# haoheliu/AudioLDM2

Measured on AMD Instinct MI355X. Metric: audio_seconds_per_second, higher is better.
Workload: dtype f32 storage/accumulate; each product = 6 bf16 MFMA partial products of exact 3-part operand splits (fp32-grade); 1 GPU; audioldm2-full: batch 8 prompts/GPU x 1 GPU, 10.24 s @16 kHz, 200 DDIM steps, CFG 3.5, eta 1.0, n_candidates 1; one step = sample_log + VAE decode + HiFi-GAN + D2H of the waveform; synthetic conditioning, random-init weights, host-CPU RNG noise; global_batch=8, parallelism=prompt-sharded replicas x1, weight_broadcast_bytes=0

## Files before the change

audioldm2_amd/csrc/api.hip:

```cpp
#include "common.h"
#include <string.h>

namespace aldm {
static thread_local char g_err[512] = "";
void set_error(const char* fmt, ...) {
    va_list ap;
    va_start(ap, fmt);
    vsnprintf(g_err, sizeof(g_err), fmt, ap);
    va_end(ap);
}
}

extern "C" int aldm_version(void) { return 26; }
extern "C" const char* aldm_last_error(void) { return aldm::g_err; }
```

audioldm2_amd/csrc/igemm.hip:

```cpp
#include "igemm_kernel.h"
#include <algorithm>
#include <atomic>
#include <stdlib.h>

namespace aldm {

int igemm_launch_pre0(int BM, int BN, int kgroups, bool uni, bool w8, dim3 grid, hipStream_t st, const IgemmK& p);
int igemm_launch_pre1(int BM, int BN, int kgroups, bool uni, bool w8, dim3 grid, hipStream_t st, const IgemmK& p);
int igemm_launch_pre2(int BM, int BN, int kgroups, bool uni, bool w8, dim3 grid, hipStream_t st, const IgemmK& p);
int igemm_launch_pre3(int BM, int BN, int kgroups, bool uni, bool w8, dim3 grid, hipStream_t st, const IgemmK& p);
int igemm_launch_pre4(int BM, int BN, int kgroups, bool uni, bool w8, dim3 grid, hipStream_t st, const IgemmK& p);
int igemm_launch_bx_pre0(int BM, int BN, int kgroups, bool uni, bool w8, dim3 grid, hipStream_t st, const IgemmK& p);
int igemm_launch_bx_pre1(int BM, int BN, int kgroups, bool uni, bool w8, dim3 grid, hipStream_t st, const IgemmK& p);
int igemm_launch_bx_pre2(int BM, int BN, int kgroups, bool uni, bool w8, dim3 grid, hipStream_t st, const IgemmK& p);
int igemm_launch_bx_pre3(int BM, int BN, int kgroups, bool uni, bool w8, dim3 grid, hipStream_t st, const IgemmK& p);

int igemm_launch_dma(int BM, int BN, int nst, int parts, bool f16, dim3 grid, hipStream_t st, const IgemmK& p);
bool igemm_dma_config_ok(int BM, int BN, int nst, int parts);
#ifdef ALDM_TEST_HOOKS
extern std::atomic<int> g_debug_drop_product;
#endif
int igemm_launch_dma_ws(int BM, int BN, int nst, int parts, int blocks, hipStream_t st, const IgemmK& p);
bool igemm_dma_ws_config_ok(int BM, int BN, int nst, int parts);
int igemm_dma_ws_blocks_per_cu(int BM, int BN, int nst, int parts);
// ... 58 lines not shown
        split_store4_out(d, d.out_split, orow, d.out_split_c, n, r);
    }
}

__global__ void pack_weight_kernel(const float* __restrict__ src, float* __restrict__ dst, int N,
                                   int Cin, int KH, int KW, int Kg, int Npad) {
    const int64_t total = (int64_t)Kg * Npad * 4;
    for (int64_t i = blockIdx.x * (int64_t)blockDim.x + threadIdx.x; i < total;
         i += (int64_t)gridDim.x * blockDim.x) {
        const int j = i & 3;
        const int n = (i >> 2) % Npad;
        const int kg = (i >> 2) / Npad;
        const int k = kg * 4 + j;
        float v = 0.f;
        if (n < N && k < KH * KW * Cin) {
            const int tap = k / Cin, ci = k - tap * Cin;
            const int kh = tap / KW, kw = tap - kh * KW;
            v = src[(((int64_t)n * Cin + ci) * KH + kh) * KW + kw];
        }
        dst[i] = v;
    }
}

__global__ void pack_weight_tr_kernel(const float* __restrict__ src, float* __restrict__ dst, int N,
                                      int Cin, int KWfull, int T, int phase, int stride, int Kg,
                                      int Npad) {
    const int64_t total = (int64_t)Kg * Npad * 4;
    for (int64_t i = blockIdx.x * (int64_t)blockDim.x + threadIdx.x; i < total;
         i += (int64_t)gridDim.x * blockDim.x) {
        const int jj = i & 3;
        const int n = (i >> 2) % Npad;
        const int kg = (i >> 2) / Npad;
        const int k = kg * 4 + jj;
        float v = 0.f;
        if (n < N && k < T * Cin) {
            const int kwp = k / Cin, ci = k - kwp * Cin;
            const int j = T - 1 - kwp;
            const int kk = phase + j * stride;
            if (kk < KWfull) v = src[((int64_t)ci * N + n) * KWfull + kk];
        }
        dst[i] = v;
    }
}

__global__ void pack_kn_kernel(const float* __restrict__ src, float* __restrict__ dst, int K, int N,
                               int lds, int Kg, int Npad, int64_t stride_src, int64_t stride_dst) {
// ... 98 lines not shown
    return mask < 0 ? default_wave8_mask() : mask;
}

static thread_local int g_force_mma = 0;
extern "C" int aldm_igemm_mma(int mode) {
    const int prev = g_force_mma;
    if (mode >= 0 && mode <= 2) g_force_mma = mode;
    return prev;
}

static std::atomic<int> g_epi_forms{-1};
static int epi_forms_on() {
    static const int env_on = [] {
        const char* e = getenv("ALDM_EPI_FORMS");
        return (e && e[0] == '0' && e[1] == 0) ? 0 : 1;
    }();
    const int v = g_epi_forms.load(std::memory_order_relaxed);
    return v < 0 ? env_on : v;
}
extern "C" int aldm_igemm_epilogue_forms(int on) {
    const int prev = epi_forms_on();
    g_epi_forms.store(on == 0 || on == 1 ? on : -1, std::memory_order_relaxed);
    return prev;
}

static int plan_epilogue_form(const IgemmK& p, int BM, int BN) {
    const aldm_igemm_desc& d = p.d;
    if (!epi_forms_on() || !p.dma || d.a_fmt != ALDM_FMT_BF16) return ALDM_EPI_FORM_GENERIC;
    const bool inst = p.ws == 0   ? igemm_dma_form_ok(BM, BN, p.nst, d.split_parts)
                      : p.ws == 2 ? igemm_dma_lw_form_ok(BM, BN, p.nst, d.split_parts)
                      : p.ws == 4 ? igemm_dma_halo_form_ok(BM, BN, p.nst, p.ws_blocks, d.split_parts, p.os_rows)
                                  : false;
    if (!inst) return ALDM_EPI_FORM_GENERIC;
    if (d.epi_mode != ALDM_EPI_PLAIN || p.splits != 1 || d.act != ALDM_ACT_NONE || d.alpha != 1.0f || d.accumulate ||
        d.out_mul > 0 || d.batch != 1)
        return ALDM_EPI_FORM_GENERIC;
    auto al16 = [](const void* q) { return (reinterpret_cast<uintptr_t>(q) & 15) == 0; };
    if ((d.N & 3) != 0 || (d.ldo & 3) != 0 || (d.stride_o & 3) != 0 || !al16(d.out) || !al16(d.res) || !al16(d.bias) ||
        !al16(d.rowbias) || (d.rowbias && (p.rb_ld & 3) != 0))
        return ALDM_EPI_FORM_GENERIC;
    if (d.out_split && (d.out_split_fmt != ALDM_FMT_BF16 || d.out_split_parts != d.split_parts)) return ALDM_EPI_FORM_GENERIC;
#ifdef ALDM_TEST_HOOKS
    if (g_debug_drop_product.load(std::memory_order_relaxed)) return ALDM_EPI_FORM_GENERIC;
#endif
    if (d.res && d.rowbias) return ALDM_EPI_FORM_GENERIC;
    return d.res ? ALDM_EPI_FORM_RES : (d.rowbias ? ALDM_EPI_FORM_ROWBIAS : ALDM_EPI_FORM_PLAIN);
// ... 40 lines not shown
    if (d.rowbias || d.accumulate || d.act != ALDM_ACT_NONE) return false;
    auto al16 = [](const void* q) { return (reinterpret_cast<uintptr_t>(q) & 15) == 0; };
    if ((d.N & 3) != 0 || (d.ldo & 3) != 0 || !al16(d.out) || !al16(d.res)) return false;
    return true;
}

static int dma_halo_chunks(const IgemmK& p, int BM) {
    const aldm_igemm_desc& d = p.d;
    if (d.KH != 3 || d.KW != 3 || d.SH != 1 || d.SW != 1 || d.PH != 1 || d.PW != 1 || d.DH != 1 || d.DW != 1) return 0;
    if (d.up_h != 1 || d.up_w != 1 || d.OH != d.H || d.OW != d.W || d.out_mul > 0 || d.batch > 1) return 0;
    if (d.W <= 0 || (d.W & (d.W - 1)) != 0 || BM % d.W != 0 || p.OHW % BM != 0) return 0;
    return ((BM / d.W + 2) * d.W + 15) / 16;
}

static bool tile_supported(int BM, int BN) {
    return (BM == 128 && (BN == 128 || BN == 64 || BN == 32)) || (BM == 64 && (BN == 128 || BN == 64));
}

static int igemm_prepare(const aldm_igemm_desc* dd, IgemmK& p, int& BM, int& BN) {
    ALDM_CHECK(dd != nullptr, "aldm_igemm: null descriptor");
    p.d = *dd;
    aldm_igemm_desc& d = p.d;
    p.epi_form = ALDM_EPI_FORM_GENERIC;
    ALDM_CHECK((d.x1 || d.a_split) && d.w && (d.out || d.out_split), "aldm_igemm: null x1/w/out");
    if (!d.x1) d.x1 = reinterpret_cast<const float*>(d.a_split);
    if (d.split_parts == 0) d.split_parts = 3;
    ALDM_CHECK(d.split_parts == 2 || d.split_parts == 3, "aldm_igemm: split_parts must be 0 / 3 or 2");
    if (d.out_split_parts == 0) d.out_split_parts = d.split_parts;
    ALDM_CHECK(d.out_split_parts == 2 || d.out_split_parts == 3, "aldm_igemm: out_split_parts must be 0, 2 or 3");
    ALDM_CHECK(d.a_fmt == ALDM_FMT_BF16 || (d.a_fmt == ALDM_FMT_F16 && d.a_split != nullptr && d.split_parts == 2 && d.acc_scale > 0.0f),
               "aldm_igemm: a_fmt = ALDM_FMT_F16 needs a pre-split operand (a_split), 2-part images and acc_scale > 0");
    if (d.a_fmt == ALDM_FMT_BF16) d.acc_scale = 1.0f;
    ALDM_CHECK(d.out_split_fmt == ALDM_FMT_BF16 ||
                   (d.out_split_fmt == ALDM_FMT_F16 && d.out_split_scale > 0.0f &&
                    (d.epi_mode == ALDM_EPI_QKV ? (d.k_split != nullptr && d.vt_split != nullptr && d.vt_scale > 0.0f) : d.out_split != nullptr)),
               "aldm_igemm: out_split_fmt = ALDM_FMT_F16 needs out_split (QKV: k_split, vt_split and vt_scale) and out_split_scale > 0");
    if (d.out_split_fmt == ALDM_FMT_F16) d.out_split_parts = 2;
    if (!d.x2) d.C2 = 0;
    if (d.pix1 == 0) d.pix1 = d.C1;
    if (d.pix2 == 0) d.pix2 = d.C2;
    if (d.up_h == 0) d.up_h = 1;
    if (d.up_w == 0) d.up_w = 1;
    if (d.batch == 0) d.batch = 1;
    p.Cin = d.C1 + d.C2;
    ALDM_CHECK(d.C1 > 0 && d.C1 % 4 == 0 && d.C2 % 4 == 0,
               "aldm_igemm: C1=%d/C2=%d must be multiples of 4", d.C1, d.C2);
// ... 364 lines not shown
    if (bn) *bn = BN;
    if (flops) *flops = 2ll * p.M * p.d.N * p.d.K * p.d.batch;
    if (splits) *splits = p.splits;
    if (kgroups) *kgroups = p.kgroups;
    if (mma) *mma = p.bx ? ALDM_MMA_BF16X6 : ALDM_MMA_F32;
    return 0;
}

extern "C" int aldm_igemm_plan_stages(const aldm_igemm_desc* dd) {
    IgemmK p;
    int BM, BN;
    if (igemm_prepare(dd, p, BM, BN)) return -1;
    if (p.dma && p.ws == 4) return 400 + (BM == 128 && p.ws_blocks == 4 ? 10 : 0) + p.nst;
    return p.dma ? p.nst + 100 * p.ws : 0;
}

extern "C" int aldm_igemm_plan_epilogue(const aldm_igemm_desc* dd) {
    IgemmK p;
    int BM, BN;
    if (igemm_prepare(dd, p, BM, BN)) return -1;
    return plan_epilogue_form(p, BM, BN);
}

extern "C" int64_t aldm_igemm_ws_floats(const aldm_igemm_desc* dd) {
    if (!dd) return 0;
    aldm_igemm_desc t = *dd;
    t.ws = reinterpret_cast<float*>(uintptr_t(16));
    t.ws_floats = INT64_MAX;
    IgemmK p;
    int BM, BN;
    if (igemm_prepare(&t, p, BM, BN)) return 0;
    return p.splits > 1 ? (int64_t)p.d.batch * p.splits * p.M * p.d.N : 0;
}

extern "C" int aldm_igemm(const aldm_igemm_desc* dd, void* stream) {
    IgemmK p;
    int BM, BN;
    int rc = igemm_prepare(dd, p, BM, BN);
    if (rc) return rc;
    p.epi_form = plan_epilogue_form(p, BM, BN);
    const aldm_igemm_desc& d = p.d;
    dim3 grid((unsigned)(p.tiles_m * p.tiles_n), (unsigned)p.splits, (unsigned)d.batch);
    hipStream_t st = (hipStream_t)stream;
    const int pre = p.pre;
    const bool uni = p.OHW % BM == 0;
    const int env_w8 = g_wave8_mask < 0 ? default_wave8_mask() : g_wave8_mask;
// ... 96 lines not shown
    hipStream_t st = (hipStream_t)stream;
    if (!transposed) {
        const int K = KH * KW * Cin;
        const int Kg = (K + 3) / 4;
        const int64_t total = (int64_t)Kg * Npad * 4;
        const int blocks = (int)std::min<int64_t>(cdiv64(total, 256), 4096);
        hipLaunchKernelGGL(pack_weight_kernel, dim3(blocks), dim3(256), 0, st, src, dst, N, Cin, KH,
                           KW, Kg, Npad);
    } else {
        ALDM_CHECK(KH == 1 && stride > 0 && phase >= 0 && phase < stride,
                   "aldm_pack_weight: bad transposed args");
        const int T = (KW + stride - 1) / stride;
        const int K = T * Cin;
        const int Kg = (K + 3) / 4;
        const int64_t total = (int64_t)Kg * Npad * 4;
        const int blocks = (int)std::min<int64_t>(cdiv64(total, 256), 4096);
        hipLaunchKernelGGL(pack_weight_tr_kernel, dim3(blocks), dim3(256), 0, st, src, dst, N, Cin,
                           KW, T, phase, stride, Kg, Npad);
    }
    ALDM_LAUNCH_CHECK("aldm_pack_weight");
    return 0;
}

extern "C" int aldm_pack_kn(const float* src, float* dst, int K, int N, int lds, int batch,
                            int64_t stride_src, int64_t stride_dst, void* stream) {
    ALDM_CHECK(src && dst && K > 0 && N > 0 && lds >= N && batch > 0, "aldm_pack_kn: bad args");
    const int Npad = (N + 31) / 32 * 32;
    const int Kg = (K + 3) / 4;
    const int64_t total = (int64_t)Kg * Npad * 4;
    const int blocks = (int)std::min<int64_t>(cdiv64(total, 256), 4096);
    hipLaunchKernelGGL(pack_kn_kernel, dim3(blocks, batch), dim3(256), 0, (hipStream_t)stream, src,
                       dst, K, N, lds, Kg, Npad, stride_src, stride_dst);
    ALDM_LAUNCH_CHECK("aldm_pack_kn");
    return 0;
}
```

audioldm2_amd/lib.py:

```python
from __future__ import annotations

import ctypes as C
import os

_HERE = os.path.dirname(os.path.abspath(__file__))
LIB_PATH = os.environ.get("ALDM_LIB_PATH") or os.path.join(_HERE, "libaldm_hip.so")
ABI_VERSION = 26

ACT_NONE, ACT_SILU, ACT_LRELU, ACT_TANH, ACT_LOGCLAMP, ACT_GELU, ACT_GELU_TANH = range(7)
B_PACKED, B_NT = 0, 1
EPI_PLAIN, EPI_GEGLU, EPI_QKV = 0, 1, 2
GN_CHUNKED, GN_FUSED, GN_FUSED_SPLIT = 0, 1, 2
FMT_BF16, FMT_F16 = 0, 1
EPI_FORM_GENERIC, EPI_FORM_PLAIN, EPI_FORM_ROWBIAS, EPI_FORM_RES = range(4)


class IgemmDesc(C.Structure):

    _fields_ = [
        ("x1", C.c_void_p), ("x2", C.c_void_p),
        ("C1", C.c_int32), ("C2", C.c_int32),
        ("pix1", C.c_int32), ("pix2", C.c_int32),
        ("B", C.c_int32), ("H", C.c_int32), ("W", C.c_int32),
        ("up_h", C.c_int32), ("up_w", C.c_int32),
        ("KH", C.c_int32), ("KW", C.c_int32), ("SH", C.c_int32), ("SW", C.c_int32),
        ("PH", C.c_int32), ("PW", C.c_int32), ("DH", C.c_int32), ("DW", C.c_int32),
        ("OH", C.c_int32), ("OW", C.c_int32),
        ("pre_scale", C.c_void_p), ("pre_shift", C.c_void_p),
        ("pre_act", C.c_int32), ("pre_slope", C.c_float),
        ("w", C.c_void_p),
        ("b_mode", C.c_int32), ("ldb", C.c_int32),
        ("K", C.c_int32), ("N", C.c_int32),
        ("bias", C.c_void_p), ("rowbias", C.c_void_p), ("res", C.c_void_p), ("out", C.c_void_p),
        ("ldo", C.c_int32), ("act", C.c_int32), ("act_slope", C.c_float), ("alpha", C.c_float),
        ("accumulate", C.c_int32),
        ("out_mul", C.c_int32), ("out_off", C.c_int32), ("out_len", C.c_int32),
        ("batch", C.c_int32),
        ("stride_x", C.c_int64), ("stride_w", C.c_int64), ("stride_o", C.c_int64),
        ("rowbias_ld", C.c_int32), ("epi_mode", C.c_int32),
        ("ws", C.c_void_p), ("ws_floats", C.c_int64),
        ("hint_bm", C.c_int32), ("hint_bn", C.c_int32), ("hint_splits", C.c_int32), ("hint_kgroups", C.c_int32),
        ("w_split", C.c_void_p), ("hint_mma", C.c_int32), ("hint_stages", C.c_int32),
        ("a_split", C.c_void_p), ("out_split", C.c_void_p), ("out_split_c", C.c_int32), ("split_parts", C.c_int32),
        ("out_split_act", C.c_int32), ("out_split_slope", C.c_float),
        ("k_split", C.c_void_p), ("vt_split", C.c_void_p), ("qkv_c", C.c_int32), ("qkv_rows", C.c_int32),
        ("a_fmt", C.c_int32), ("acc_scale", C.c_float), ("out_split_parts", C.c_int32),
        ("out_split_fmt", C.c_int32), ("out_split_scale", C.c_float), ("vt_scale", C.c_float),
    ]


MAX_WINDOWS = 32


class WindowStarts(C.Structure):

    _fields_ = [("n", C.c_int), ("s", C.c_int * MAX_WINDOWS)]


MAX_ROWS = 64


class WindowRows(C.Structure):

    _fields_ = [("n", C.c_int), ("s", C.c_int * MAX_ROWS)]


_SIGS = {
    "aldm_version": (C.c_int, []),
    "aldm_last_error": (C.c_char_p, []),
    "aldm_igemm": (C.c_int, [C.POINTER(IgemmDesc), C.c_void_p]),
    "aldm_igemm_plan": (C.c_int, [C.POINTER(IgemmDesc), C.POINTER(C.c_int), C.POINTER(C.c_int),
                                  C.POINTER(C.c_int64), C.POINTER(C.c_int), C.POINTER(C.c_int),
                                  C.POINTER(C.c_int)]),
    "aldm_igemm_ws_floats": (C.c_int64, [C.POINTER(IgemmDesc)]),
    "aldm_igemm_plan_stages": (C.c_int, [C.POINTER(IgemmDesc)]),
    "aldm_igemm_plan_epilogue": (C.c_int, [C.POINTER(IgemmDesc)]),
    "aldm_igemm_epilogue_forms": (C.c_int, [C.c_int]),
    "aldm_igemm_force": (None, [C.c_int, C.c_int, C.c_int, C.c_int]),
    "aldm_igemm_force_stages": (None, [C.c_int]),
    "aldm_igemm_wave8_mask": (C.c_int, [C.c_int]),
    "aldm_split_image_bytes": (C.c_int64, [C.c_int64, C.c_int, C.c_int]),
    "aldm_split_rows": (C.c_int, [C.c_void_p, C.c_void_p, C.c_int, C.c_int, C.c_int64, C.c_int, C.c_void_p, C.c_void_p,
                                  C.c_int, C.c_void_p, C.c_void_p, C.c_int, C.c_void_p]),
    "aldm_split_rows_act": (C.c_int, [C.c_void_p, C.c_void_p, C.c_int, C.c_int, C.c_int64, C.c_int, C.c_void_p, C.c_void_p,
                                      C.c_int, C.c_float, C.c_void_p, C.c_void_p, C.c_int, C.c_void_p]),
    "aldm_layernorm_split": (C.c_int, [C.c_void_p, C.c_void_p, C.c_void_p, C.c_int, C.c_int, C.c_void_p, C.c_void_p,
                                       C.c_float, C.c_int, C.c_void_p]),
    "aldm_attention_d32_split": (C.c_int, [C.c_void_p, C.c_void_p, C.c_void_p, C.c_void_p, C.c_void_p, C.c_int, C.c_int,
                                           C.c_int, C.c_int, C.c_int, C.c_int, C.c_int, C.c_int, C.c_int,
                                           C.c_void_p, C.c_float, C.c_void_p]),
    "aldm_split_bytes_parts": (C.c_int64, [C.c_int, C.c_int, C.c_int]),
    "aldm_pack_split_bf16_parts": (C.c_int, [C.c_void_p, C.c_void_p, C.c_int, C.c_int, C.c_int, C.c_void_p]),
    "aldm_pack_split_f16": (C.c_int, [C.c_void_p, C.c_void_p, C.c_int, C.c_int, C.c_float, C.c_void_p]),
    "aldm_split_rows_f16": (C.c_int, [C.c_void_p, C.c_void_p, C.c_int, C.c_int, C.c_int64, C.c_int, C.c_void_p, C.c_void_p,
                                      C.c_int, C.c_float, C.c_void_p, C.c_void_p, C.c_int, C.c_float, C.c_void_p]),
    "aldm_groupnorm_split_f16": (C.c_int, [C.c_void_p, C.c_void_p, C.c_int, C.c_int, C.c_int, C.c_int, C.c_int, C.c_float,
                                           C.c_void_p, C.c_void_p, C.c_int, C.c_void_p, C.c_void_p, C.c_void_p, C.c_void_p,
                                           C.c_void_p, C.c_int, C.c_float, C.c_void_p]),
    "aldm_layernorm_split_f16": (C.c_int, [C.c_void_p, C.c_void_p, C.c_void_p, C.c_int, C.c_int, C.c_void_p, C.c_void_p,
                                           C.c_float, C.c_float, C.c_void_p]),
# ... 199 lines not shown
```

audioldm2_amd/ops.py:

```python
from __future__ import annotations

import ctypes as C
import json
import os
from dataclasses import dataclass
from typing import List, Optional, Sequence, Tuple

import torch

from . import lib as _l
from .lib import (ACT_GELU, ACT_GELU_TANH, ACT_LOGCLAMP, ACT_LRELU, ACT_NONE, ACT_SILU, ACT_TANH, B_NT, B_PACKED,
                  IgemmDesc)


def _stream() -> int:
    return torch.cuda.current_stream().cuda_stream


def _p(t: Optional[torch.Tensor]):
    return None if t is None else t.data_ptr()


def _chk(t: torch.Tensor, name: str):
    if not (t.is_cuda and t.dtype == torch.float32 and t.is_contiguous()):
# ... 88 lines not shown


def _norm_f16_scale(gamma: torch.Tensor, beta: Optional[torch.Tensor], n: int) -> float:
    import math
    return _pow2_scale(math.sqrt(float(n)) * _absmax_cached(gamma) + _absmax_cached(beta))


@dataclass
class Packed:
    data: torch.Tensor
    N: int
    Cin: int
    KH: int
    KW: int
    bias: Optional[torch.Tensor] = None
    split: Optional[torch.Tensor] = None
    split2: Optional[torch.Tensor] = None
    split16: Optional[torch.Tensor] = None
    w_scale: float = 0.0
    cmax: Optional[float] = None
    bmax: float = 0.0
    geglu: bool = False
    halves: Optional[tuple] = None

    @property
    def K(self) -> int:
        return self.KH * self.KW * self.Cin

    def out_bound(self, rn: float) -> float:
        if self.cmax is None:
            if torch.cuda.is_current_stream_capturing():
                raise RuntimeError("f16x3: a weight's column norms must be known before graph capture (run one eager step)")
            npad = self.data.numel() // (4 * ((self.K + 3) // 4))
            self.cmax = float(self.data.view(-1, npad, 4).double().pow(2).sum((0, 2)).max().sqrt())
            self.bmax = 0.0 if self.bias is None else float(self.bias.abs().max())
        return rn * self.cmax + self.bmax

    def geglu_bound(self, rn: float, rt: float) -> Tuple[float, float]:
        import math
        assert self.geglu
        if self.halves is None:
            if torch.cuda.is_current_stream_capturing():
                raise RuntimeError("f16x3: a weight's column norms must be known before graph capture (run one eager step)")
            npad = self.data.numel() // (4 * ((self.K + 3) // 4))
            cn = self.data.view(-1, npad, 4).double().pow(2).sum((0, 2)).sqrt()[:self.N].view(-1, 2, 32)
            b = torch.zeros(self.N, device=self.data.device) if self.bias is None else self.bias
            b = b.double().view(-1, 2, 32)
            self.halves = tuple((float(cn[:, j].max()), float(cn[:, j].median()), float(b[:, j].abs().max()),
                                 float(b[:, j].pow(2).mean().sqrt())) for j in range(2))
        bound, typ = 1.0, 1.0
# ... 145 lines not shown


def _workspace(lib, d: IgemmDesc, device) -> None:
    need = lib.aldm_igemm_ws_floats(C.byref(d))
    if need <= 0:
        return
    key = (device.index if device.index is not None else torch.cuda.current_device(), WS_SLOT)
    buf = _ws.get(key)
    if buf is None or buf.numel() < need:
        if torch.cuda.is_current_stream_capturing():
            return
        if buf is not None:
            _ws_retired.append(buf)
        buf = torch.empty(max(need, 8 << 20), device=device, dtype=torch.float32)
        _ws[key] = buf
    d.ws = buf.data_ptr()
    d.ws_floats = buf.numel()


_TUNE_FIELDS = ("B", "H", "W", "C1", "C2", "pix1", "up_h", "up_w", "KH", "KW", "SH", "SW", "PH", "PW", "DH", "DW",
                "OH", "OW", "N", "b_mode", "batch", "epi_mode", "out_mul")
_TUNED = None
TUNE_LOG = None


def tune_key(d: IgemmDesc) -> str:
    return ",".join(str(getattr(d, f)) for f in _TUNE_FIELDS) + f",{_pre_mode(d)}" + \
        (("," + ("dma2" if d.split_parts == 2 else "dma")) if d.a_split else "")


def _tuned_table(bx=False):
    global _TUNED
    if _TUNED is None:
        _TUNED = {False: {}, True: {}, "dma": {}, "dma2": {}}
        if os.environ.get("ALDM_NO_TUNING", "0") != "1":
            for mode, name in ((False, "mi355x_igemm.json"), (True, "mi355x_igemm_bf16x6.json"),
                               ("dma", "mi355x_igemm_dma.json"), ("dma2", "mi355x_igemm_dma_bf16x3.json")):
                path = os.path.join(os.environ.get("ALDM_TUNING_DIR", ""), name)
                if not (os.environ.get("ALDM_TUNING_DIR") and os.path.exists(path)):
                    path = os.path.join(os.path.dirname(os.path.abspath(__file__)), "tuning", name)
                if os.path.exists(path):
                    with open(path) as f:
                        _TUNED[mode] = {k: v[:5] if mode is True else v[:4] for k, v in json.load(f)["entries"].items()}
    return _TUNED[bx]


def _set_split_operand(d: IgemmDesc, x: "SplitT", pw: "Packed", so: Optional["SplitT"] = None) -> None:
    d.a_split = x.data_ptr()
    d.split_parts = x.parts
    if x.fmt == "f16":
# ... 125 lines not shown
    global _wave8_mask
    _wave8_mask = mask
    return _l.load().aldm_igemm_wave8_mask(mask)


def _npad(n: int) -> int:
    return (n + 31) // 32 * 32


def pack_conv(weight: torch.Tensor, bias: Optional[torch.Tensor] = None) -> Packed:
    w = weight.detach().to(device="cuda", dtype=torch.float32).contiguous()
    if w.dim() == 2:
        N, Cin, KH, KW = w.shape[0], w.shape[1], 1, 1
    elif w.dim() == 3:
        N, Cin, KH, KW = w.shape[0], w.shape[1], 1, w.shape[2]
    else:
        N, Cin, KH, KW = w.shape
    K = KH * KW * Cin
    dst = torch.empty(((K + 3) // 4) * _npad(N) * 4, device="cuda", dtype=torch.float32)
    lib = _l.load()
    _l.check(lib.aldm_pack_weight(w.data_ptr(), dst.data_ptr(), N, Cin, KH, KW, 0, 0, 1, _stream()),
             "pack_weight")
    b = None if bias is None else bias.detach().to(device="cuda", dtype=torch.float32).contiguous()
    return Packed(dst, N, Cin, KH, KW, b)


def pack_geglu(weight: torch.Tensor, bias: Optional[torch.Tensor]) -> Packed:
    two_inner = weight.shape[0]
    inner = two_inner // 2
    assert weight.dim() == 2 and two_inner % 64 == 0
    g = torch.arange(inner // 32).view(-1, 1, 1)
    j = torch.arange(2).view(1, -1, 1)
    l = torch.arange(32).view(1, 1, -1)
    perm = (j * inner + g * 32 + l).reshape(-1).to(weight.device)
    pw = pack_conv(weight.detach()[perm], None if bias is None else bias.detach()[perm])
    pw.geglu = True
    return pw


def linear_geglu(x, pw: Packed, split_out: Optional[str] = None, gate_act: int = ACT_NONE,
                 out: Optional[torch.Tensor] = None):
    is_split = isinstance(x, SplitT)
    if not is_split:
        _chk(x, "linear_geglu.x")
    shp = x.shape
    M = (x.rows if is_split else x.numel() // shp[-1])
    assert shp[-1] == pw.Cin and pw.KH == 1 and pw.KW == 1 and pw.N % 64 == 0
# ... 168 lines not shown
        OH = (VH + 2 * pad[0] - dil[0] * (pw.KH - 1) - 1) // stride[0] + 1
        OW = (VW + 2 * pad[1] - dil[1] * (pw.KW - 1) - 1) // stride[1] + 1
    else:
        OH, OW = out_hw
    N = pw.N
    if remap is not None:
        out_mul, out_off, out_len = remap
        oshape = (B, 1, out_len, N)
    else:
        out_mul = out_off = out_len = 0
        oshape = (B, OH, OW, N)
    if split_out == "only":
        assert out is None and not accumulate
    elif out is None:
        assert not accumulate
        out = torch.empty(oshape, device=x.device, dtype=torch.float32)
    else:
        _chk(out, "conv.out")
        assert out.numel() == oshape[0] * oshape[1] * oshape[2] * oshape[3], (out.shape, oshape)
    so = SplitT.empty(oshape, x.device) if split_out else None
    if bias is None and use_pw_bias:
        bias = pw.bias
    d = IgemmDesc()
    if is_split:
        _set_split_operand(d, x, pw, so)
    else:
        d.x1 = x.data_ptr(); d.split_parts = so.parts if so is not None else 3
    d.x2 = _p(x2)
    d.C1 = C1; d.C2 = C2; d.pix1 = 0; d.pix2 = 0
    d.B = B; d.H = H; d.W = W; d.up_h = up[0]; d.up_w = up[1]
    d.KH = pw.KH; d.KW = pw.KW; d.SH = stride[0]; d.SW = stride[1]
    d.PH = pad[0]; d.PW = pad[1]; d.DH = dil[0]; d.DW = dil[1]
    d.OH = OH; d.OW = OW
    if pre is not None:
        d.pre_scale = pre[0].data_ptr(); d.pre_shift = pre[1].data_ptr()
    d.pre_act = pre_act; d.pre_slope = pre_slope
    d.w = pw.data.data_ptr(); d.b_mode = B_PACKED; d.ldb = 0
    if not is_split:
        d.w_split = pw.split_ptr(3)
    d.K = pw.K; d.N = N
    d.bias = _p(bias); d.rowbias = _p(rowbias); d.res = _p(res); d.out = _p(out)
    if so is not None:
        d.out_split = so.data_ptr(); d.out_split_c = N
        d.out_split_act = split_act; d.out_split_slope = split_slope
    if rowbias is not None:
        if not (rowbias.dim() == 2 and rowbias.stride(1) == 1 and rowbias.shape == (B, N)):
            raise RuntimeError("conv.rowbias: need a [B, N] fp32 view with unit inner stride")
        d.rowbias_ld = rowbias.stride(0)
    d.ldo = N; d.act = act; d.act_slope = act_slope; d.alpha = alpha
    d.accumulate = 1 if accumulate else 0
    d.out_mul = out_mul; d.out_off = out_off; d.out_len = out_len
    d.batch = 1
    _igemm(d, "igemm(conv)")
    if split_out == "only":
        return so
    return (out.view(oshape), so) if split_out else out.view(oshape)


def linear(x, pw: Packed, **kw):
    shp = x.shape
    if isinstance(x, SplitT):
        M = x.rows
        y = conv(x.view(1, 1, M, shp[-1]), pw, **kw)
    else:
        M = x.numel() // shp[-1]
        y = conv(x.reshape(1, 1, M, shp[-1]), pw, **kw)
    oshape = (*shp[:-1], pw.N)
    if isinstance(y, tuple):
        return y[0].view(oshape), y[1].view(oshape)
    return y.view(oshape)


def _view3(t: torch.Tensor, name: str):
    if not (t.is_cuda and t.dtype == torch.float32 and t.dim() == 3 and t.stride(2) == 1):
        raise RuntimeError(f"{name}: need a [Z, R, D] fp32 CUDA view with unit inner stride")
# ... 990 lines not shown
```

audioldm2_amd/unet.py:

```python
from __future__ import annotations

from typing import List, Optional

import torch
import torch.nn as nn

import os

from . import ops
from .ops import ACT_NONE, ACT_SILU

PRESPLIT_ATTENTION = os.environ.get("ALDM_ATTN_PRESPLIT", "1") != "0" and "ALDM_ATTN_MMA" not in os.environ


class ResBlock(nn.Module):

    def __init__(self, channels, emb_channels, dropout, out_channels=None):
        super().__init__()
        self.channels = channels
        self.out_channels = out_channels or channels
        self.in_layers = nn.Sequential(nn.GroupNorm(32, channels), nn.SiLU(),
                                       nn.Conv2d(channels, self.out_channels, 3, padding=1))
        self.emb_layers = nn.Sequential(nn.SiLU(), nn.Linear(emb_channels, self.out_channels))
        self.out_layers = nn.Sequential(nn.GroupNorm(32, self.out_channels), nn.SiLU(), nn.Dropout(p=dropout),
# ... 390 lines not shown
    def collect_context_kv(self, contexts):
        out = []
        for m in self.modules():
            if isinstance(m, BasicTransformerBlock) and m._kv:
                for ctx, _ver, kv, fold in m._kv:
                    if any(ctx is c for c in contexts):
                        out.append((m, ctx, kv, fold))
        return out

    def refresh_context_kv(self, entries):
        n = 0
        for m, ctx, kv, fold in entries:
            pk = m._prepare()
            ops.linear(ctx, pk["kv2"], out=kv)
            if fold is not None:
                fold.prepare(kv, pk["wq2"], pk["wout2"])
            m._kv = [(ctx, ctx._version, kv, fold)] + [c for c in (m._kv or ()) if c[2] is not kv][:1]
            n += 1
        return n

    def _prepare(self):
        if self._pk is None:
            f = lambda t: t.detach().float().cuda().contiguous()
            rbs = [m for m in self.modules() if isinstance(m, ResBlock)]
            off = 0
            for m in rbs:
                m._emb_slice = slice(off, off + m.out_channels)
                off += m.out_channels
            self._pk = dict(
                emb_all=ops.pack_conv(torch.cat([m.emb_layers[1].weight for m in rbs], 0),
                                      torch.cat([m.emb_layers[1].bias for m in rbs], 0)),
                te0=ops.pack_conv(self.time_embed[0].weight, self.time_embed[0].bias),
                te2=ops.pack_conv(self.time_embed[2].weight, self.time_embed[2].bias),
                film=ops.pack_conv(self.film_emb.weight, self.film_emb.bias)
                if self.use_extra_film_by_concat else None,
                gn=(f(self.out[0].weight), f(self.out[0].bias)),
                out=ops.pack_conv(self.out[2].weight, self.out[2].bias),
            )
        return self._pk

    def _shared_prefix_end(self, context_list):
        if self.use_extra_film_by_concat:
            return None
        for bi, blk in enumerate(self.input_blocks):
            st = 0
            for li, layer in enumerate(blk):
                if isinstance(layer, SpatialTransformer):
                    if st >= 1 and st - 1 < len(context_list) and context_list[st - 1] is not None:
                        return bi, li
                    st += 1
        return None

    @torch.no_grad()
    def forward(self, x, timesteps=None, y=None, context_list=None, context_attn_mask_list=None, cfg_shared=False, **kwargs):
        assert (y is not None) == self.use_extra_film_by_concat, \
            "must specify y if and only if the model is class-conditional or film embedding conditional"
        if not x.is_cuda:
            raise RuntimeError("UNetModel(HIP) runs on the MI355X only; there is no CPU path")
        pk = self._prepare()
        context_list = [c.float().contiguous() if c is not None else None for c in (context_list or [])]
        mask_list = list(context_attn_mask_list or [])
        div = self._shared_prefix_end(context_list) if cfg_shared else None
        B = x.shape[0]
        if cfg_shared:
            assert timesteps.shape[0] in (B, 2 * B) and all(c is None or c.shape[0] == 2 * B for c in context_list), \
                "cfg_shared: x [B, ...] once, contexts for the 2B rows [uncond ; cond]"
            timesteps = timesteps[:B]
            if div is None:
                x = x.repeat(2, 1, 1, 1)
                timesteps = timesteps.repeat(2)
        t_emb = ops.timestep_embedding(timesteps, self.model_channels)
        emb = ops.linear(ops.linear(t_emb, pk["te0"], act=ACT_SILU), pk["te2"])
        if self.use_extra_film_by_concat:
            emb = torch.cat([emb, ops.linear(y.float().contiguous(), pk["film"])], dim=-1).contiguous()
        emb_rows = ops.linear(emb, pk["emb_all"], pre_act=ACT_SILU)
        emb = _EmbSlices(emb_rows)
        h = ops.nchw_to_nhwc(x.float().contiguous())
        hs = []
        if div is None:
            for module in self.input_blocks:
                h = module.run(h, emb, context_list, mask_list)
                hs.append(h)
        else:
            dup = lambda t: t.repeat(2, *([1] * (t.dim() - 1)))
            emb_half, emb = emb, _EmbSlices(dup(emb_rows))
            for bi, module in enumerate(self.input_blocks):
                if bi < div[0]:
                    h = module.run(h, emb_half, context_list, mask_list)
                elif bi == div[0]:
                    h = module.run(h, emb_half, context_list, mask_list, hi=div[1])
                    h = module.run(dup(h), emb, context_list, mask_list, lo=div[1])
                else:
                    h = module.run(h, emb, context_list, mask_list)
                hs.append(h)
        h = self.middle_block.run(h, emb, context_list, mask_list)
        for module in self.output_blocks:
            skip = hs.pop()
            if skip.shape[0] != h.shape[0]:
# ... 6 lines not shown
```

include/aldm_hip.h:

```cpp
#ifndef ALDM_HIP_H
#define ALDM_HIP_H

#include <stdint.h>

#ifdef __cplusplus
extern "C" {
#endif

int aldm_version(void);
const char* aldm_last_error(void);

enum {
    ALDM_ACT_NONE = 0,
    ALDM_ACT_SILU = 1,
    ALDM_ACT_LRELU = 2,
    ALDM_ACT_TANH = 3,
    ALDM_ACT_LOGCLAMP = 4,
    ALDM_ACT_GELU = 5,
    ALDM_ACT_GELU_TANH = 6
};

enum { ALDM_EPI_PLAIN = 0, ALDM_EPI_GEGLU = 1, ALDM_EPI_QKV = 2 };

enum {
// ... 37 lines not shown
    float* ws;
    int64_t ws_floats;
    int32_t hint_bm, hint_bn, hint_splits;
    int32_t hint_kgroups;
    const void* w_split;
    int32_t hint_mma;
    int32_t hint_stages;
    const void* a_split;
    void* out_split;
    int32_t out_split_c;
    int32_t split_parts;
    int32_t out_split_act;
    float out_split_slope;
    void* k_split;
    void* vt_split;
    int32_t qkv_c;
    int32_t qkv_rows;
    int32_t a_fmt;
    float acc_scale;
    int32_t out_split_parts;
    int32_t out_split_fmt;
    float out_split_scale;
    float vt_scale;
} aldm_igemm_desc;

int aldm_igemm(const aldm_igemm_desc* d, void* stream);
int64_t aldm_igemm_ws_floats(const aldm_igemm_desc* d);
enum { ALDM_FMT_BF16 = 0, ALDM_FMT_F16 = 1 };
int aldm_igemm_plan(const aldm_igemm_desc* d, int* bm, int* bn, int64_t* flops, int* splits, int* kgroups,
                    int* mma);
int aldm_igemm_plan_stages(const aldm_igemm_desc* d);
enum { ALDM_EPI_FORM_GENERIC = 0, ALDM_EPI_FORM_PLAIN = 1, ALDM_EPI_FORM_ROWBIAS = 2, ALDM_EPI_FORM_RES = 3 };
int aldm_igemm_plan_epilogue(const aldm_igemm_desc* d);
int aldm_igemm_epilogue_forms(int on);
void aldm_igemm_force(int bm, int bn, int splits, int kgroups);
void aldm_igemm_force_stages(int stages);
int aldm_igemm_wave8_mask(int mask);
int aldm_igemm_mma(int mode);
#ifdef ALDM_TEST_HOOKS
int aldm_debug_drop_product(int on);
#endif
int64_t aldm_split_bytes(int K, int N);
int aldm_pack_split_bf16(const float* packed, void* dst, int K, int N, void* stream);
int64_t aldm_split_bytes_parts(int K, int N, int parts);
int aldm_pack_split_bf16_parts(const float* packed, void* dst, int K, int N, int parts, void* stream);
int aldm_pack_split_f16(const float* packed, void* dst, int K, int N, float scale, void* stream);

int64_t aldm_split_image_bytes(int64_t rows, int C, int parts);
int aldm_split_rows(const float* x1, const float* x2, int C1, int C2, int64_t rows, int P, const float* scale,
                    const float* shift, int act, void* dst, void* dst_raw, int parts, void* stream);
int aldm_split_rows_act(const float* x1, const float* x2, int C1, int C2, int64_t rows, int P, const float* scale,
                        const float* shift, int act, float slope, void* dst, void* dst_raw, int parts, void* stream);
int aldm_split_rows_f16(const float* x1, const float* x2, int C1, int C2, int64_t rows, int P, const float* scale,
                        const float* shift, int act, float slope, void* dst, void* dst_raw, int raw_parts, float f16_scale,
                        void* stream);

int aldm_pack_weight(const float* src, float* dst, int N, int Cin, int KH, int KW,
// ... 164 lines not shown
```

Baseline: 19.55 audio-s/s.

## Merge width-2 3x3 convolutions into 1-wide GEMMs with column-merged weights

For 3x3 stride-1 convs whose input width is 2, the two output columns are folded into the output-channel dimension. A new packed weight image of shape 6*Cin by 2N (zero padding taps dropped) lets the implicit GEMM run as a 1-wide conv with half the K-padding waste and doubled N. The per-ResBlock embedding projection is duplicated to produce [B,2N] row biases that match the merged layout. It adds extra weight images and a geometry blacklist, and requires a warm-up eager step before graph capture.

```diff
diff --git a/audioldm2_amd/csrc/api.hip b/audioldm2_amd/csrc/api.hip
--- a/audioldm2_amd/csrc/api.hip
+++ b/audioldm2_amd/csrc/api.hip
@@ -11,5 +11,5 @@
 }
 }
 
-extern "C" int aldm_version(void) { return 26; }
+extern "C" int aldm_version(void) { return 27; }
 extern "C" const char* aldm_last_error(void) { return aldm::g_err; }
diff --git a/audioldm2_amd/csrc/igemm.hip b/audioldm2_amd/csrc/igemm.hip
--- a/audioldm2_amd/csrc/igemm.hip
+++ b/audioldm2_amd/csrc/igemm.hip
@@ -104,6 +104,30 @@
     }
 }
 
+__host__ __device__ inline int64_t wmerge_src_index(int N, int Cin, int dy, int xin, int ci, int xout, int co) {
+    (void)N;
+    const int kw = xin - xout + 1;
+    return (((int64_t)co * Cin + ci) * 3 + dy) * 3 + kw;
+}
+
+__global__ void pack_weight_wmerge_kernel(const float* __restrict__ src, float* __restrict__ dst, int N, int Cin, int Kg, int Npad) {
+    const int64_t total = (int64_t)Kg * Npad * 4;
+    for (int64_t i = blockIdx.x * (int64_t)blockDim.x + threadIdx.x; i < total; i += (int64_t)gridDim.x * blockDim.x) {
+        const int j = i & 3;
+        const int n = (i >> 2) % Npad;
+        const int kg = (i >> 2) / Npad;
+        const int k = kg * 4 + j;
+        float v = 0.f;
+        if (n < 2 * N && k < 6 * Cin) {
+            const int tap = k / Cin, ci = k - tap * Cin;
+            const int dy = tap >> 1, xin = tap & 1;
+            const int xout = n / N, co = n - xout * N;
+            v = src[wmerge_src_index(N, Cin, dy, xin, ci, xout, co)];
+        }
+        dst[i] = v;
+    }
+}
+
 __global__ void pack_weight_tr_kernel(const float* __restrict__ src, float* __restrict__ dst, int N,
                                       int Cin, int KWfull, int T, int phase, int stride, int Kg,
                                       int Npad) {
@@ -248,6 +272,57 @@
     const int prev = epi_forms_on();
     g_epi_forms.store(on == 0 || on == 1 ? on : -1, std::memory_order_relaxed);
     return prev;
+}
+
+static std::atomic<int> g_conv_wmerge{-1};
+static int conv_wmerge_on() {
+    static const int env_on = [] {
+        const char* e = getenv("ALDM_CONV_WMERGE");
+        return (e && e[0] == '0' && e[1] == 0) ? 0 : 1;
+    }();
+    const int v = g_conv_wmerge.load(std::memory_order_relaxed);
+    return v < 0 ? env_on : v;
+}
+extern "C" int aldm_conv_wmerge(int on) {
+    const int prev = conv_wmerge_on();
+    g_conv_wmerge.store(on == 0 || on == 1 ? on : -1, std::memory_order_relaxed);
+    return prev;
+}
+
+static bool wmerge_geometry_wins(int H, int C2x, int N2x) {
+    (void)H;
+    if (N2x == 1280 && (C2x == 768 || C2x == 1280 || C2x == 2048 || C2x == 2560)) return false;
+    return true;
+}
+extern "C" int aldm_conv_wmerge_wins(int H, int C, int N) {
+    return conv_wmerge_on() && H > 0 && C > 0 && N > 0 && C % 32 == 0 && wmerge_geometry_wins(H, 2 * C, 2 * N) ? 1 : 0;
+}
+
+static bool wmerge_applies(const aldm_igemm_desc& d) {
+    if (!conv_wmerge_on() || !d.a_split || !d.wm_split || d.a_fmt != ALDM_FMT_BF16) return false;
+    if (d.W != 2 || d.OW != 2 || d.KH != 3 || d.KW != 3 || d.SH != 1 || d.SW != 1 || d.DH != 1 || d.DW != 1 || d.PW != 1) return false;
+    if (d.up_h > 1 || d.up_w > 1 || d.OH != d.H + 2 * d.PH - 2 || d.OH < 1) return false;
+    if (d.x2 || d.C2 != 0 || d.pre_scale || d.pre_shift || d.pre_act != ALDM_ACT_NONE) return false;
+    if (d.out_mul > 0 || d.accumulate || d.out_split || d.epi_mode != ALDM_EPI_PLAIN || d.batch > 1) return false;
+    if (d.C1 <= 0 || d.C1 % 32 != 0 || (d.pix1 != 0 && d.pix1 != d.C1) || d.K != 9 * d.C1 || d.N <= 0 || d.ldo != d.N) return false;
+    if (d.b_mode != ALDM_B_PACKED || (reinterpret_cast<uintptr_t>(d.wm_split) & 15) != 0) return false;
+    if (d.bias && !d.wm_bias) return false;
+    if (d.rowbias && (!d.wm_rowbias2 || d.rowbias_ld < 2 * d.N)) return false;
+    return wmerge_geometry_wins(d.H, 2 * d.C1, 2 * d.N);
+}
+
+static void wmerge_rewrite(aldm_igemm_desc& d) {
+    d.K = 6 * d.C1;
+    d.C1 *= 2;
+    d.pix1 = 0;
+    d.W = 1;
+    d.OW = 1;
+    d.KW = 1;
+    d.PW = 0;
+    d.N *= 2;
+    d.ldo = d.N;
+    d.bias = d.bias ? d.wm_bias : nullptr;
+    d.w_split = d.wm_split;
 }
 
 static int plan_epilogue_form(const IgemmK& p, int BM, int BN) {
@@ -334,6 +409,7 @@
     p.d = *dd;
     aldm_igemm_desc& d = p.d;
     p.epi_form = ALDM_EPI_FORM_GENERIC;
+    if (wmerge_applies(d)) wmerge_rewrite(d);
     ALDM_CHECK((d.x1 || d.a_split) && d.w && (d.out || d.out_split), "aldm_igemm: null x1/w/out");
     if (!d.x1) d.x1 = reinterpret_cast<const float*>(d.a_split);
     if (d.split_parts == 0) d.split_parts = 3;
@@ -744,6 +820,19 @@
     return plan_epilogue_form(p, BM, BN);
 }
 
+extern "C" int aldm_igemm_plan_wmerge(const aldm_igemm_desc* dd) {
+    IgemmK p;
+    int BM, BN;
+    if (igemm_prepare(dd, p, BM, BN)) return -1;
+    return wmerge_applies(*dd) ? 1 : 0;
+}
+
+extern "C" int64_t aldm_conv_wmerge_index(int N, int Cin, int dy, int xin, int ci, int xout, int co) {
+    if (N <= 0 || Cin <= 0 || dy < 0 || dy > 2 || xin < 0 || xin > 1 || xout < 0 || xout > 1 || ci < 0 || ci >= Cin || co < 0 || co >= N)
+        return -1;
+    return wmerge_src_index(N, Cin, dy, xin, ci, xout, co);
+}
+
 extern "C" int64_t aldm_igemm_ws_floats(const aldm_igemm_desc* dd) {
     if (!dd) return 0;
     aldm_igemm_desc t = *dd;
@@ -886,6 +975,17 @@
     return 0;
 }
 
+extern "C" int aldm_pack_weight_wmerge(const float* src, float* dst, int N, int Cin, void* stream) {
+    ALDM_CHECK(src && dst && N > 0 && Cin > 0 && (int64_t)N * Cin * 9 < (1ll << 31), "aldm_pack_weight_wmerge: bad args");
+    const int Npad = (2 * N + 31) / 32 * 32;
+    const int Kg = (6 * Cin + 3) / 4;
+    const int64_t total = (int64_t)Kg * Npad * 4;
+    const int blocks = (int)std::min<int64_t>(cdiv64(total, 256), 4096);
+    hipLaunchKernelGGL(pack_weight_wmerge_kernel, dim3(blocks), dim3(256), 0, (hipStream_t)stream, src, dst, N, Cin, Kg, Npad);
+    ALDM_LAUNCH_CHECK("aldm_pack_weight_wmerge");
+    return 0;
+}
+
 extern "C" int aldm_pack_kn(const float* src, float* dst, int K, int N, int lds, int batch,
                             int64_t stride_src, int64_t stride_dst, void* stream) {
     ALDM_CHECK(src && dst && K > 0 && N > 0 && lds >= N && batch > 0, "aldm_pack_kn: bad args");
diff --git a/audioldm2_amd/lib.py b/audioldm2_amd/lib.py
--- a/audioldm2_amd/lib.py
+++ b/audioldm2_amd/lib.py
@@ -5,7 +5,7 @@
 
 _HERE = os.path.dirname(os.path.abspath(__file__))
 LIB_PATH = os.environ.get("ALDM_LIB_PATH") or os.path.join(_HERE, "libaldm_hip.so")
-ABI_VERSION = 26
+ABI_VERSION = 27
 
 ACT_NONE, ACT_SILU, ACT_LRELU, ACT_TANH, ACT_LOGCLAMP, ACT_GELU, ACT_GELU_TANH = range(7)
 B_PACKED, B_NT = 0, 1
@@ -46,6 +46,7 @@
         ("k_split", C.c_void_p), ("vt_split", C.c_void_p), ("qkv_c", C.c_int32), ("qkv_rows", C.c_int32),
         ("a_fmt", C.c_int32), ("acc_scale", C.c_float), ("out_split_parts", C.c_int32),
         ("out_split_fmt", C.c_int32), ("out_split_scale", C.c_float), ("vt_scale", C.c_float),
+        ("wm_split", C.c_void_p), ("wm_bias", C.c_void_p), ("wm_rowbias2", C.c_int32),
     ]
 
 
@@ -76,6 +77,11 @@
     "aldm_igemm_plan_stages": (C.c_int, [C.POINTER(IgemmDesc)]),
     "aldm_igemm_plan_epilogue": (C.c_int, [C.POINTER(IgemmDesc)]),
     "aldm_igemm_epilogue_forms": (C.c_int, [C.c_int]),
+    "aldm_igemm_plan_wmerge": (C.c_int, [C.POINTER(IgemmDesc)]),
+    "aldm_conv_wmerge": (C.c_int, [C.c_int]),
+    "aldm_conv_wmerge_wins": (C.c_int, [C.c_int, C.c_int, C.c_int]),
+    "aldm_conv_wmerge_index": (C.c_int64, [C.c_int] * 7),
+    "aldm_pack_weight_wmerge": (C.c_int, [C.c_void_p, C.c_void_p, C.c_int, C.c_int, C.c_void_p]),
     "aldm_igemm_force": (None, [C.c_int, C.c_int, C.c_int, C.c_int]),
     "aldm_igemm_force_stages": (None, [C.c_int]),
     "aldm_igemm_wave8_mask": (C.c_int, [C.c_int]),
diff --git a/audioldm2_amd/ops.py b/audioldm2_amd/ops.py
--- a/audioldm2_amd/ops.py
+++ b/audioldm2_amd/ops.py
@@ -134,10 +134,34 @@
     bmax: float = 0.0
     geglu: bool = False
     halves: Optional[tuple] = None
+    src: Optional[torch.Tensor] = None
+    wm: Optional[dict] = None
+    wm_bias: Optional[torch.Tensor] = None
 
     @property
     def K(self) -> int:
         return self.KH * self.KW * self.Cin
+
+    def wmerge_ptr(self, parts: int = 3) -> int:
+        if self.wm is None:
+            self.wm = {}
+        img = self.wm.get(parts)
+        if img is None:
+            if torch.cuda.is_current_stream_capturing():
+                raise RuntimeError("a weight's column-merged split image must exist before graph capture (run one eager step)")
+            assert self.src is not None and tuple(self.src.shape) == (self.N, self.Cin, 3, 3)
+            lib = _l.load()
+            w = self.src.detach().to(device=self.data.device, dtype=torch.float32).contiguous()
+            K2, N2 = 6 * self.Cin, 2 * self.N
+            packed = torch.empty(((K2 + 3) // 4) * _npad(N2) * 4, device=w.device, dtype=torch.float32)
+            _l.check(lib.aldm_pack_weight_wmerge(w.data_ptr(), packed.data_ptr(), self.N, self.Cin, _stream()), "pack_weight_wmerge")
+            img = torch.empty(lib.aldm_split_bytes_parts(K2, N2, parts) // 4, device=w.device, dtype=torch.int32)
+            _l.check(lib.aldm_pack_split_bf16_parts(packed.data_ptr(), img.data_ptr(), K2, N2, parts, _stream()),
+                     "pack_split_bf16(wmerge)")
+            self.wm[parts] = img
+            if self.bias is not None and self.wm_bias is None:
+                self.wm_bias = torch.cat([self.bias, self.bias]).contiguous()
+        return img.data_ptr()
 
     def out_bound(self, rn: float) -> float:
         if self.cmax is None:
@@ -329,10 +353,14 @@
                 "OH", "OW", "N", "b_mode", "batch", "epi_mode", "out_mul")
 _TUNED = None
 TUNE_LOG = None
+WMERGE_LOG = None
 
 
 def tune_key(d: IgemmDesc) -> str:
-    return ",".join(str(getattr(d, f)) for f in _TUNE_FIELDS) + f",{_pre_mode(d)}" + \
+    g = {f: getattr(d, f) for f in _TUNE_FIELDS}
+    if d.wm_split:
+        g.update(W=1, OW=1, C1=2 * d.C1, KW=1, PW=0, N=2 * d.N)
+    return ",".join(str(g[f]) for f in _TUNE_FIELDS) + f",{_pre_mode(d)}" + \
         (("," + ("dma2" if d.split_parts == 2 else "dma")) if d.a_split else "")
 
 
@@ -504,7 +532,19 @@
     _l.check(lib.aldm_pack_weight(w.data_ptr(), dst.data_ptr(), N, Cin, KH, KW, 0, 0, 1, _stream()),
              "pack_weight")
     b = None if bias is None else bias.detach().to(device="cuda", dtype=torch.float32).contiguous()
-    return Packed(dst, N, Cin, KH, KW, b)
+    return Packed(dst, N, Cin, KH, KW, b, src=weight.detach() if (KH, KW) == (3, 3) and weight.dim() == 4 else None)
+
+
+def conv_wmerge(on: int = -1) -> int:
+    return _l.load().aldm_conv_wmerge(on)
+
+
+def conv_wmerge_wins(H: int, C: int, N: int) -> bool:
+    return bool(_l.load().aldm_conv_wmerge_wins(H, C, N))
+
+
+def conv_wmerge_index(N: int, Cin: int, dy: int, xin: int, ci: int, xout: int, co: int) -> int:
+    return _l.load().aldm_conv_wmerge_index(N, Cin, dy, xin, ci, xout, co)
 
 
 def pack_geglu(weight: torch.Tensor, bias: Optional[torch.Tensor]) -> Packed:
@@ -719,7 +759,10 @@
     if bias is None and use_pw_bias:
         bias = pw.bias
     d = IgemmDesc()
-    if is_split:
+    wm_cand = (is_split and x.fmt == "bf16" and pw.src is not None and W == 2 and so is None and (bias is None or bias is pw.bias))
+    if wm_cand:
+        d.a_split = x.data_ptr(); d.split_parts = x.parts
+    elif is_split:
         _set_split_operand(d, x, pw, so)
     else:
         d.x1 = x.data_ptr(); d.split_parts = so.parts if so is not None else 3
@@ -740,14 +783,30 @@
     if so is not None:
         d.out_split = so.data_ptr(); d.out_split_c = N
         d.out_split_act = split_act; d.out_split_slope = split_slope
+    rb_wide = False
     if rowbias is not None:
-        if not (rowbias.dim() == 2 and rowbias.stride(1) == 1 and rowbias.shape == (B, N)):
-            raise RuntimeError("conv.rowbias: need a [B, N] fp32 view with unit inner stride")
+        rb_wide = rowbias.dim() == 2 and tuple(rowbias.shape) == (B, 2 * N)
+        if not (rowbias.dim() == 2 and rowbias.stride(1) == 1 and (rowbias.shape == (B, N) or rb_wide)):
+            raise RuntimeError("conv.rowbias: need a [B, N] (or duplicated [B, 2N]) fp32 view with unit inner stride")
         d.rowbias_ld = rowbias.stride(0)
     d.ldo = N; d.act = act; d.act_slope = act_slope; d.alpha = alpha
     d.accumulate = 1 if accumulate else 0
     d.out_mul = out_mul; d.out_off = out_off; d.out_len = out_len
     d.batch = 1
+    if wm_cand:
+        d.wm_split = d.w_split = 16
+        d.wm_bias = 16 if bias is not None else None
+        d.wm_rowbias2 = 1 if rb_wide else 0
+        if _l.load().aldm_igemm_plan_wmerge(C.byref(d)) == 1:
+            d.wm_split = pw.wmerge_ptr(x.parts); d.w_split = None
+            d.wm_bias = _p(pw.wm_bias) if bias is not None else None
+        else:
+            d.wm_split = None; d.wm_bias = None; d.wm_rowbias2 = 0
+            d.w_split = pw.split_ptr(x.parts)
+    if WMERGE_LOG is not None:
+        q = IgemmDesc.from_buffer_copy(d)
+        q.wm_split = 16; q.wm_bias = 16 if bias is not None else None; q.wm_rowbias2 = 1 if rb_wide else 0
+        WMERGE_LOG.append((_l.load().aldm_igemm_plan_wmerge(C.byref(q)), bool(d.wm_split)))
     _igemm(d, "igemm(conv)")
     if split_out == "only":
         return so
diff --git a/audioldm2_amd/unet.py b/audioldm2_amd/unet.py
--- a/audioldm2_amd/unet.py
+++ b/audioldm2_amd/unet.py
@@ -436,14 +436,17 @@
     def _prepare(self):
         if self._pk is None:
             f = lambda t: t.detach().float().cuda().contiguous()
-            rbs = [m for m in self.modules() if isinstance(m, ResBlock)]
-            off = 0
-            for m in rbs:
-                m._emb_slice = slice(off, off + m.out_channels)
-                off += m.out_channels
+            ds = 1
+            for blk in list(self.input_blocks) + [self.middle_block] + list(self.output_blocks):
+                for layer in blk:
+                    if isinstance(layer, ResBlock):
+                        layer._ds = ds
+                    elif isinstance(layer, Downsample):
+                        ds *= 2
+                    elif isinstance(layer, Upsample):
+                        ds //= 2
             self._pk = dict(
-                emb_all=ops.pack_conv(torch.cat([m.emb_layers[1].weight for m in rbs], 0),
-                                      torch.cat([m.emb_layers[1].bias for m in rbs], 0)),
+                emb_all={},
                 te0=ops.pack_conv(self.time_embed[0].weight, self.time_embed[0].bias),
                 te2=ops.pack_conv(self.time_embed[2].weight, self.time_embed[2].bias),
                 film=ops.pack_conv(self.film_emb.weight, self.film_emb.bias)
@@ -452,6 +455,24 @@
                 out=ops.pack_conv(self.out[2].weight, self.out[2].bias),
             )
         return self._pk
+
+    def _emb_all(self, lat_h, lat_w):
+        rbs = [m for m in self.modules() if isinstance(m, ResBlock)]
+        wide = tuple(lat_w % m._ds == 0 and lat_w // m._ds == 2 and ops.use_dma() and
+                     ops.conv_wmerge_wins(max(lat_h // m._ds, 1), m.channels, m.out_channels) for m in rbs)
+        ent = self._pk["emb_all"].get(wide)
+        if ent is None:
+            ws, bs, slices, off = [], [], [], 0
+            for m, twice in zip(rbs, wide):
+                n = m.out_channels * (2 if twice else 1)
+                ws += [m.emb_layers[1].weight] * (2 if twice else 1)
+                bs += [m.emb_layers[1].bias] * (2 if twice else 1)
+                slices.append(slice(off, off + n))
+                off += n
+            ent = self._pk["emb_all"][wide] = (ops.pack_conv(torch.cat(ws, 0), torch.cat(bs, 0)), slices)
+        for m, sl in zip(rbs, ent[1]):
+            m._emb_slice = sl
+        return ent[0]
 
     def _shared_prefix_end(self, context_list):
         if self.use_extra_film_by_concat:
@@ -487,7 +508,7 @@
         emb = ops.linear(ops.linear(t_emb, pk["te0"], act=ACT_SILU), pk["te2"])
         if self.use_extra_film_by_concat:
             emb = torch.cat([emb, ops.linear(y.float().contiguous(), pk["film"])], dim=-1).contiguous()
-        emb_rows = ops.linear(emb, pk["emb_all"], pre_act=ACT_SILU)
+        emb_rows = ops.linear(emb, self._emb_all(x.shape[-2], x.shape[-1]), pre_act=ACT_SILU)
         emb = _EmbSlices(emb_rows)
         h = ops.nchw_to_nhwc(x.float().contiguous())
         hs = []
diff --git a/include/aldm_hip.h b/include/aldm_hip.h
--- a/include/aldm_hip.h
+++ b/include/aldm_hip.h
@@ -83,6 +83,9 @@
     int32_t out_split_fmt;
     float out_split_scale;
     float vt_scale;
+    const void* wm_split;
+    const float* wm_bias;
+    int32_t wm_rowbias2;
 } aldm_igemm_desc;
 
 int aldm_igemm(const aldm_igemm_desc* d, void* stream);
@@ -94,6 +97,11 @@
 enum { ALDM_EPI_FORM_GENERIC = 0, ALDM_EPI_FORM_PLAIN = 1, ALDM_EPI_FORM_ROWBIAS = 2, ALDM_EPI_FORM_RES = 3 };
 int aldm_igemm_plan_epilogue(const aldm_igemm_desc* d);
 int aldm_igemm_epilogue_forms(int on);
+int aldm_igemm_plan_wmerge(const aldm_igemm_desc* d);
+int aldm_conv_wmerge(int on);
+int aldm_conv_wmerge_wins(int H, int C, int N);
+int64_t aldm_conv_wmerge_index(int N, int Cin, int dy, int xin, int ci, int xout, int co);
+int aldm_pack_weight_wmerge(const float* src, float* dst, int N, int Cin, void* stream);
 void aldm_igemm_force(int bm, int bn, int splits, int kgroups);
 void aldm_igemm_force_stages(int stages);
 int aldm_igemm_wave8_mask(int mask);
```

Result: no change. 19.54 audio-s/s (median of 2 runs) (-0.0%).
